# TheShinning/gps-sdr-sim

Hardware: AMD Instinct MI355X
Metric: IQ MSamples/s (and × real-time) at 2.6 MS/s, 12 sats, -b 16; 1/2/4/8 GPU (higher is better)
Workload: dtype int64 phases + f16 x f16 -> f32 MFMA accumulate (exact integer sums)

## Files before the change

### gps-sdr-sim_amd/csrc/common/gss_lin.h

```cpp
#ifndef GSS_LIN_H
#define GSS_LIN_H

#include <stdint.h>

#ifndef GSS_LIN_CH
#define GSS_LIN_CH     16
#endif
#define GSS_LIN_CHUNK  (64 * GSS_LIN_CH)
#define GSS_LIN_SEG    4096

#if defined(__HIPCC__)
#define GSS_LIN_FN static __host__ __device__ inline
#else
#define GSS_LIN_FN static inline
#endif

#define GSS_LIN_CSH    26

GSS_LIN_FN uint32_t gss_lin_dx(uint64_t xs) { return (uint32_t)((xs * 64u + (1ull << 31)) >> 32); }
GSS_LIN_FN uint32_t gss_lin_dz(uint64_t zs)
{
    return (uint32_t)((zs * 64u + (1ull << (GSS_LIN_CSH - 1))) >> GSS_LIN_CSH);
}
GSS_LIN_FN uint64_t gss_lin_xa(uint64_t xs)
{
    const int64_t e = (int64_t)(((uint64_t)gss_lin_dx(xs) << 32) - xs * 64u);
    return (1ull << 31) - (uint64_t)((e * (GSS_LIN_CH - 1)) / 2);
}
GSS_LIN_FN uint64_t gss_lin_za(uint64_t zs)
{
    const int64_t ec = (int64_t)(((uint64_t)gss_lin_dz(zs) << GSS_LIN_CSH) - zs * 64u);
    return (1ull << (GSS_LIN_CSH - 1)) - (uint64_t)((ec * (GSS_LIN_CH - 1)) / 2);
}

GSS_LIN_FN uint32_t gss_lin_e0(uint64_t chips)
{
    const uint32_t e = (uint32_t)(chips % 1023u);
    return e ? e : 1023u;
}

#define GSS_LIN_KDEV_CARR(zs)                                                                      \
    ((((uint64_t)GSS_LIN_CH / 2 + 3) << 31) +                                                     \
     ((2 + (((uint64_t)gss_lin_dz(zs) * (GSS_LIN_CH - 1)) >> 32)) << 32))
#define GSS_LIN_KDEV_CODE (((uint64_t)GSS_LIN_CH / 2 + 3) << (GSS_LIN_CSH - 1))
#define GSS_LIN_WIN_OK(zs) ((zs) * 63u + (3ull << 50) <= (31ull << 50))

#define GSS_LIN_TWE     2560
#define GSS_LIN_CBW_PRE 2
GSS_LIN_FN uint32_t gss_lin_wstep16(int n_per_blk)
{
    return (uint32_t)((104755200ull + (uint64_t)n_per_blk / 2) / (uint64_t)n_per_blk);
}
GSS_LIN_FN int gss_lin_win16_ok(uint64_t zs, int n_per_blk)
{
    const int64_t U = (int64_t)1 << 50, z = (int64_t)zs;
    const int64_t kd = (int64_t)GSS_LIN_KDEV_CODE + ((int64_t)1 << 27);
    const uint32_t w = gss_lin_wstep16(n_per_blk);
    if (zs == 0 || zs >= (uint64_t)U)
        return 0;
    for (int s = 0; s < GSS_LIN_CH; s++) {
        const int64_t f = (int64_t)(((uint64_t)s * w) >> 4) - GSS_LIN_CBW_PRE;
        if (64 * s * z - kd < f * U)
            return 0;
        if (U + (64 * s + 63) * z + kd > (f + 32) * U)
            return 0;
    }
    return 1025 * U + (int64_t)(GSS_LIN_SEG - GSS_LIN_CHUNK) * z + kd < (int64_t)GSS_LIN_TWE * U;
}

GSS_LIN_FN uint64_t gss_lin_lane(uint64_t xs, uint64_t zs, uint32_t l)
{
    const uint32_t lx = (uint32_t)(((uint64_t)l * xs + (1ull << 31)) >> 32);
    const uint32_t lz = (uint32_t)(((uint64_t)l * zs) >> GSS_LIN_CSH);
    return ((uint64_t)lx << 32) | lz;
}

typedef struct {
    int cell, chip;
} gss_lin_kc;

GSS_LIN_FN gss_lin_kc gss_lin_kernel_at(uint64_t x0, uint64_t xs, uint64_t z0, uint64_t zs,
                                         int64_t p)
{
    const int64_t c = p & ~(int64_t)(GSS_LIN_CHUNK - 1);
    const int64_t l = p & 63, s = (p - c) >> 6;
    const uint64_t lane = gss_lin_lane(xs, zs, (uint32_t)l);
    const int64_t n0 = p & ~(int64_t)(GSS_LIN_SEG - 1);
    const unsigned __int128 zn = (unsigned __int128)z0 + (unsigned __int128)(uint64_t)n0 * zs;
    const int64_t chips = (int64_t)(zn >> 50), e0 = gss_lin_e0((uint64_t)chips);
    const __int128 z = (__int128)z0 + (__int128)c * (__int128)zs -
                      (__int128)(chips - e0) * ((__int128)1 << 50);
    const unsigned __int128 zk = (unsigned __int128)((z + (int64_t)gss_lin_za(zs)) >> GSS_LIN_CSH);
    const uint64_t za = (uint64_t)(uint32_t)zk + (uint32_t)lane;
    const uint64_t zw = (uint64_t)(uint32_t)za + (uint64_t)s * gss_lin_dz(zs);
    const unsigned __int128 kz = zk + (uint32_t)lane + (unsigned __int128)(uint64_t)s *
                                 gss_lin_dz(zs);
    const uint32_t xb = (uint32_t)((x0 + (uint64_t)c * xs + gss_lin_xa(xs)) >> 32);
    const uint32_t xk = xb + (uint32_t)(lane >> 32) + (uint32_t)(za >> 32) +
                        (uint32_t)s * gss_lin_dx(xs) + (uint32_t)(zw >> 32);
    gss_lin_kc r;
    r.cell = (int)(xk >> 23);
    r.chip = (int)((uint64_t)(kz >> 24) % 1023u);
    return r;
}

#endif
```

### gps-sdr-sim_amd/csrc/hip/gss_synth.hip

```cpp
#include <hip/hip_runtime.h>
#include <stdint.h>
#include <stdlib.h>
#include <string.h>
#include "gpssim_amd.h"
#include "../common/gss_phase.h"
#include "../common/gss_lin.h"

#define SYNTH_THREADS  256
#define SYNTH_WAVES    (SYNTH_THREADS / 64)
#define ANCHOR_THREADS 64
#define CHUNK_BYTES    128
#define CHUNK_PIECES   (CHUNK_BYTES / 16)
#define LUT_N          1024

struct lut_arg { int16_t sin512[512]; int16_t cos512[512]; };

__global__ __launch_bounds__(ANCHOR_THREADS) void gss_anchor_kernel(
    const gss_chan_blk_t *__restrict__ blk, const int32_t *__restrict__ nch,
    const double *__restrict__ carr_ck, int nblk, int nchp, int n_per_blk, int nseg, int nsegp,
    int seg_r, double *__restrict__ seg_carr, double *__restrict__ seg_code,
    uint32_t *__restrict__ seg_cnt, double *__restrict__ carr_end,
    const int32_t *__restrict__ blist)
{
    const int nsub = carr_ck ? GSS_NCK : 1;
// ... 336 lines not shown
                if (src_full) {
                    uint8_t *sdst = dst + (ptrdiff_t)(src - lane) * ((ptrdiff_t)seg_r * BPS4 / 4) +
                                    (size_t)ch * CHUNK_BYTES + piece * 16;
                    const uint32_t *sp = stg + src * (CHUNK_BYTES / 4) + piece * 4;
                    store16(sdst, make_uint4(sp[0], sp[1], sp[2], sp[3]));
                }
            }
            wave_sync_lds();
        }
        if (!full && nsamp > 0) {
            int nbytes = nsamp * BPS4 / 4;
            uint8_t *bp = dst + (size_t)ch * CHUNK_BYTES;
            const uint8_t *sp = (const uint8_t *)mine;
            for (int i = 0; i < nbytes; i++)
                bp[i] = sp[i];
        }
    }
    if (bad && status)
        atomicOr(status, bad);
}

#define LIN_THREADS 256
#define LIN_WAVES   (LIN_THREADS / 64)
#define LIN_STEPS   (GSS_LIN_SEG / 64)
#define LIN_CH      GSS_LIN_CH
#define CBW_PRE     2
#define CBW_CHIPS   3072
#define CAB_W       ((CBW_CHIPS + 96) / 32)
static_assert(LIN_STEPS % LIN_CH == 0 && (LIN_CH & (LIN_CH - 1)) == 0, "whole chunks");
#define LIN_SW_SGPRS 68
typedef _Float16 lin_half4 __attribute__((ext_vector_type(4)));
typedef _Float16 lin_half8 __attribute__((ext_vector_type(8)));
typedef float lin_f4 __attribute__((ext_vector_type(4)));
#define LIN_GS    2
#define LIN_MAGF  (12582912.0f + 64.0f * LIN_GS)
#define LIN_MAGB  0x4B400000u

struct alignas(16) lin_ct {
    uint64_t B;
    uint64_t D;
    int32_t g;
    int32_t gd;
    int32_t pos1;
    uint32_t flags;
    uint32_t q0, dq, tab;
    uint32_t wa;
    uint32_t na, nb;
    uint32_t wn;
    uint32_t g2;
    uint32_t A[5][2];
};
static_assert(offsetof(lin_ct, A) % 8 == 0, "lin_ct.A: 8-byte reads");

struct lin_chan {
    uint64_t xs, zs;
    uint64_t d;
    uint32_t dq;
    uint32_t tab;
};
struct lin_seg {
    uint64_t x;
    uint64_t z;
    int32_t g01;
    int32_t pos1;
    uint32_t npatch;
    uint32_t pad;
};

__global__ void gss_linseg_kernel(const gss_lin_t *__restrict__ lin,
                                  const gss_chan_blk_t *__restrict__ blk,
                                  const int32_t *__restrict__ nch, const int32_t *__restrict__ fast,
                                  int nblk, int nseg, lin_seg *__restrict__ seg_out,
                                  lin_chan *__restrict__ chan_out)
{
    const int i = blockIdx.x * blockDim.x + threadIdx.x;
    if (i >= nblk * GSS_MAXCH * nseg)
        return;
    const int sg = i % nseg, bk = i / nseg, b = bk / GSS_MAXCH, k = bk % GSS_MAXCH;
    if (!fast[b] || k >= nch[b])
        return;
    const gss_lin_t *L = lin + bk;
    const uint64_t xa = gss_lin_xa(L->xs);
    if (sg == 0) {
        lin_chan c;
        c.xs = L->xs;
        c.zs = L->zs;
        c.d = ((uint64_t)gss_lin_dx(L->xs) << 32) | gss_lin_dz(L->zs);
        c.dq = (uint32_t)((L->zs * 64u) >> 46);
        c.tab = (uint32_t)blk[bk].ca_tbl;
        chan_out[bk] = c;
    }
    const uint64_t n0 = (uint64_t)sg * (64 * LIN_STEPS);
    const uint64_t lo = L->z0 + n0 * L->zs;
    const uint64_t hi = __umul64hi(n0, L->zs) + (lo < L->z0 ? 1u : 0u);
    const uint32_t E0 = gss_lin_e0((hi << 14) | (lo >> 50));
    lin_seg r;
    r.z = (((uint64_t)E0 << 50) | (lo & ((1ull << 50) - 1))) + gss_lin_za(L->zs);
    r.x = L->x0 + n0 * L->xs + xa;
    int q = 0;
    while (q + 1 < GSS_NGC && L->gpos[q + 1] <= (int)n0)
        q++;
    const int g0 = L->gval[q];
    const bool more = q + 1 < GSS_NGC && L->gpos[q + 1] < (int)n0 + 64 * LIN_STEPS;
    const int g1 = more ? L->gval[q + 1] : g0;
    r.g01 = (int32_t)(((uint32_t)g0 & 0xFFFFu) | ((uint32_t)g1 << 16));
    r.pos1 = more ? L->gpos[q + 1] : INT32_MAX;
    int np = 0;
    for (int j = 0; j < GSS_NPATCH; j++)
        np += L->ppos[j] >= (int)n0 && L->ppos[j] < (int)n0 + 64 * LIN_STEPS;
    r.npatch = (uint32_t)np;
    r.pad = 0;
    seg_out[i] = r;
}

__global__ void gss_cab_kernel(const uint32_t *__restrict__ ca_bits, int n_ca,
                               uint32_t *__restrict__ cab)
{
    const int i = blockIdx.x * blockDim.x + threadIdx.x;
    if (i >= n_ca * CAB_W)
        return;
    const int row = i / CAB_W, j0 = (i - row * CAB_W) * 32 - 32;
    const uint32_t *cb = ca_bits + (size_t)row * GSS_CA_WORDS;
    uint32_t w = 0;
    for (int q = 0; q < 32; q++) {
        const int e = j0 + q, chip = ((e % GSS_CA_LEN) + GSS_CA_LEN) % GSS_CA_LEN;
        w |= (((cb[chip >> 5] >> (chip & 31)) & 1u) ^ 1u) << q;
    }
    cab[i] = w;
}

__global__ void gss_tw16_kernel(const uint32_t *__restrict__ cab, int n_ca, uint32_t w,
                                uint32_t *__restrict__ tw)
{
    const int i = blockIdx.x * blockDim.x + threadIdx.x;
    if (i >= n_ca * GSS_LIN_TWE * LIN_CH)
        return;
    const int row = i / (GSS_LIN_TWE * LIN_CH), r = i - row * (GSS_LIN_TWE * LIN_CH);
    const int E = r / LIN_CH, st = r % LIN_CH;
    const uint32_t j = min((uint32_t)(E + (int)(((uint32_t)st * w) >> 4) - GSS_LIN_CBW_PRE + 32),
                           (uint32_t)(32 * CAB_W - 64));
    const uint32_t *c = cab + (size_t)row * CAB_W;
    const uint32_t lin = __builtin_amdgcn_alignbit(c[(j >> 5) + 1], c[j >> 5], j & 31);
    tw[i] = __builtin_amdgcn_alignbit(lin, lin, (32u - j) & 31u);
}

struct lin_wsrc {
    const uint32_t *W;
};

__device__ __forceinline__ void lin_wissue(const lin_wsrc &w, uint32_t (&ws)[LIN_CH])
{
#pragma unroll
    for (int s = 0; s < LIN_CH; s++)
        ws[s] = w.W[s];
}

__device__ __forceinline__ void lin_wfence(const uint32_t (&ws)[LIN_CH])
{
    static_assert(LIN_CH == 16, "the fence below names 16 windows");
    asm volatile("" :: "s"(ws[0]), "s"(ws[1]), "s"(ws[2]), "s"(ws[3]), "s"(ws[4]), "s"(ws[5]),
                 "s"(ws[6]), "s"(ws[7]), "s"(ws[8]), "s"(ws[9]), "s"(ws[10]), "s"(ws[11]),
                 "s"(ws[12]), "s"(ws[13]), "s"(ws[14]), "s"(ws[15]));
}

__device__ __forceinline__ lin_wsrc lin_wsrc_of(const lin_ct &t, const uint32_t *__restrict__ tw)
{
// ... 120 lines not shown
}

template <bool FIRST>
__device__ __forceinline__ void lin_sw_pair(lin_f4 (&cq)[LIN_CH / 2], lin_f4 c0, const lin_ct *T, int k0,
                                            int nc, int lane, const uint64_t *s_lane, uint32_t M,
                                            const int32_t *__restrict__ s_lut,
                                            const uint32_t *__restrict__ tw, uint32_t cls,
                                            bool more)
{
    const lin_ct &ta = T[k0], &tb = T[k0 + 1];
    uint64_t Pa = s_lane[k0 * 64 + lane] + ta.B, Pb = s_lane[(k0 + 1) * 64 + lane] + tb.B;
    const uint64_t Da = ta.D, Db = tb.D;
    const uint2 ga = *(const uint2 *)ta.A[cls], gb = *(const uint2 *)tb.A[cls];
    const lin_half8 A = __builtin_bit_cast(lin_half8, make_uint4(ga.x, ga.y, gb.x, gb.y));
    uint32_t na = ta.na, nb = ta.nb;
    asm volatile("" : "+v"(na), "+v"(nb));
    uint32_t wsa[LIN_CH], wsb[LIN_CH];
    lin_sw_take_a(wsa);
    lin_sw_take(wsb);
    if (k0 + 2 < nc || more)
        lin_sw_load2(tw, na, nb);
    uint32_t ea0 = 0, eb0 = 0;
#pragma unroll
    for (int s = 0; s < LIN_CH; s++) {
        uint32_t ta_, tb_;
        asm("v_lshrrev_b32_sdwa %0, %1, %2 dst_sel:DWORD dst_unused:UNUSED_PAD src0_sel:BYTE_3 "
            "src1_sel:DWORD" : "=v"(ta_) : "v"((uint32_t)Pa), "s"(wsa[s]));
        asm("v_lshrrev_b32_sdwa %0, %1, %2 dst_sel:DWORD dst_unused:UNUSED_PAD src0_sel:BYTE_3 "
            "src1_sel:DWORD" : "=v"(tb_) : "v"((uint32_t)Pb), "s"(wsb[s]));
        const uint32_t aa = __builtin_amdgcn_alignbit(ta_, (uint32_t)(Pa >> 32), 21) & M;
        const uint32_t ab = __builtin_amdgcn_alignbit(tb_, (uint32_t)(Pb >> 32), 21) & M;
        const uint32_t ea = *(const uint32_t *)((const char *)s_lut + aa);
        const uint32_t eb = *(const uint32_t *)((const char *)s_lut + ab);
        if (s & 1) {
            const uint4 bb = make_uint4(ea0, ea, eb0, eb);
            cq[s / 2] = __builtin_amdgcn_mfma_f32_16x16x32_f16(A, __builtin_bit_cast(lin_half8, bb),
                                                              FIRST ? c0 : cq[s / 2], 0, 0, 0);
        } else {
            ea0 = ea;
            eb0 = eb;
        }
        Pa += Da;
        Pb += Db;
    }
}

__device__ __forceinline__ lin_half4 lin_gain_operand(uint32_t gh, int lane)
{
    const uint32_t x = gh << ((lane & 1) * 16);
    const uint2 v = (lane & 2) ? make_uint2(0u, x) : make_uint2(x, 0u);
    return __builtin_bit_cast(lin_half4, v);
}

__device__ __forceinline__ uint32_t lin_f16_bits(int g)
{
    return (uint32_t)__builtin_bit_cast(uint16_t, (_Float16)(float)g);
}

__device__ __forceinline__ void lin_put(uint32_t *p, uint32_t v)
{
    __builtin_nontemporal_store(v, p);
}

extern "C" __device__ int gss_writelane(int, int, int) __asm("llvm.amdgcn.writelane.i32");

__device__ __forceinline__ uint32_t lin_ib(const lin_f4 (&cq)[LIN_CH / 2], int s)
{
    return __float_as_uint(cq[s / 2][2 * (s & 1)]);
}
__device__ __forceinline__ uint32_t lin_qb(const lin_f4 (&cq)[LIN_CH / 2], int s)
{
    return __float_as_uint(cq[s / 2][2 * (s & 1) + 1]);
}
__device__ __forceinline__ uint32_t lin_w16(const lin_f4 (&cq)[LIN_CH / 2], int s)
{
    const uint32_t pq = __builtin_amdgcn_perm(lin_qb(cq, s), lin_ib(cq, s), 0x06050201u);
    uint32_t r;
    asm("v_pk_add_u16 %0, %1, %2" : "=v"(r) : "v"(pq), "s"(0xC000C000u));
    return r;
}
__device__ __forceinline__ uint32_t lin_w8(const lin_f4 (&cq)[LIN_CH / 2], int s)
{
    constexpr uint32_t sh = 12u;
    uint32_t d = lin_ib(cq, s) >> sh;
    asm("v_lshrrev_b32_sdwa %0, %1, %2 dst_sel:BYTE_1 dst_unused:UNUSED_PRESERVE src0_sel:DWORD "
        "src1_sel:DWORD" : "+v"(d) : "v"(sh), "v"(lin_qb(cq, s)));
    return d;
}
__device__ __forceinline__ bool lin_ipos(const lin_f4 (&cq)[LIN_CH / 2], int s)
{
    return lin_ib(cq, s) >= LIN_MAGB + 128u * LIN_GS;
}
__device__ __forceinline__ bool lin_qpos(const lin_f4 (&cq)[LIN_CH / 2], int s)
{
    return lin_qb(cq, s) >= LIN_MAGB + 128u * LIN_GS;
}

template <int FMT, bool TAIL>
__device__ __forceinline__ void lin_store(const lin_f4 (&acc)[LIN_CH / 2], uint8_t *__restrict__ ob,
                                          int nb0, int lane, int n_per_blk)
{
    static_assert(FMT != 1 || LIN_CH == 16, "-b 1 packing assumes 16-step chunks");
    uint32_t pk[LIN_CH];
    pk[0] = 0;
#pragma unroll
    for (int s = 0; s < LIN_CH; s++) {
        const int nb = nb0 + s * 64, p = nb + lane;
// ... 40 lines not shown
                if (first + 4 * b < n_per_blk)
                    dst[b] = (uint8_t)(y >> (8 * b));
        }
    }
    if (FMT == 16) {
        __builtin_amdgcn_sched_barrier(0);
        if (!TAIL) {
            uint32_t *base = (uint32_t *)ob + nb0;
            const uint32_t off = (uint32_t)lane * 4u;
#pragma unroll
            for (int s = 0; s < LIN_CH; s++)
                asm volatile("global_store_dword %0, %1, %2 offset:%3 nt"
                             : : "v"(off), "v"(pk[s]), "s"(base + (s >> 4) * 1024),
                               "i"((s & 15) * 256) : "memory");
        } else {
#pragma unroll
            for (int s = 0; s < LIN_CH; s++) {
                const int p = nb0 + s * 64 + lane;
                if (!TAIL || p < n_per_blk)
                    lin_put(((uint32_t *)ob) + p, pk[s]);
            }
        }
    }
}

__device__ __forceinline__ void lin_patch_fix(lin_f4 (&cq)[LIN_CH / 2],
                                              const gss_lin_t *__restrict__ Lk, int nb0, int lane)
{
    for (int j = 0; j < GSS_NPATCH; j++) {
        const int pp = Lk->ppos[j];
        if (pp >= nb0 + 64 * LIN_CH)
            break;
        if (pp < nb0)
            continue;
        const int q = pp - nb0;
        const int64_t d = lane == (q & 63) ? Lk->pdelta[j] : 0;
        const int di = (int)((uint32_t)d << 10) >> 10;
        const float fi = (float)(di * LIN_GS), fq = (float)((int)((d - di) >> 22) * LIN_GS);
        const int sq = __builtin_amdgcn_readfirstlane(q >> 6);
#pragma unroll
        for (int s = 0; s < LIN_CH; s++) {
            const float m = s == sq ? 1.0f : 0.0f;
            cq[s / 2][2 * (s & 1)] = __builtin_fmaf(m, fi, cq[s / 2][2 * (s & 1)]);
            cq[s / 2][2 * (s & 1) + 1] = __builtin_fmaf(m, fq, cq[s / 2][2 * (s & 1) + 1]);
        }
    }
}


#define LIN_MINB 4
template <int FMT>
__global__ __launch_bounds__(LIN_THREADS, LIN_MINB) __attribute__((amdgpu_num_sgpr(LIN_SW_SGPRS)))
void gss_lin_kernel(
    const gss_lin_t *__restrict__ lin, const lin_seg *__restrict__ segs,
    const lin_chan *__restrict__ chans, const int32_t *__restrict__ nch,
    const int32_t *__restrict__ fast, const uint32_t *__restrict__ cab,
    const uint32_t *__restrict__ tw, lut_arg lut, int n_per_blk, int nseg, int wg_per_blk,
    uint8_t *__restrict__ out, size_t block_bytes)
{
    __shared__ int32_t s_lut[1024];
    __shared__ uint64_t s_lane[GSS_MAXCH * 64];
    __shared__ lin_ct s_ct[LIN_WAVES][GSS_MAXCH];
    const int b = blockIdx.x / wg_per_blk;
    const int w = blockIdx.x - b * wg_per_blk;
    if (!fast[b])
        return;
    const int tid = threadIdx.x, lane = tid & 63;
    const int wave = __builtin_amdgcn_readfirstlane(tid >> 6);
    for (int i = tid; i < 512; i += LIN_THREADS) {
        const uint32_t v = lin_f16_bits(lut.cos512[i]) | (lin_f16_bits(lut.sin512[i]) << 16);
        s_lut[i] = (int32_t)v;
        s_lut[512 + i] = (int32_t)(v ^ 0x80008000u);
    }
    const lin_chan *CH = chans + (size_t)b * GSS_MAXCH;
    const int nc = nch[b];
    for (int i = tid; i < nc * 64; i += LIN_THREADS)
        s_lane[i] = gss_lin_lane(CH[i >> 6].xs, CH[i >> 6].zs, (uint32_t)(i & 63));
    (void)cab;
    __syncthreads();
    uint32_t M = 0xFFCu;
    asm volatile("" : "+v"(M));
    const uint32_t cls = lin_pair_cls(lane);
    lin_f4 c0 = lin_f4{LIN_MAGF, LIN_MAGF, LIN_MAGF, LIN_MAGF};
    asm volatile("" : "+v"(c0));
    const int sg = w * LIN_WAVES + wave;
    const int n0 = sg * (64 * LIN_STEPS);
    if (n0 >= n_per_blk)
        return;
    const gss_lin_t *L = lin + (size_t)b * GSS_MAXCH;
    const lin_seg *S = segs + (size_t)b * GSS_MAXCH * nseg + sg;
    lin_ct *T = s_ct[wave];
    uint8_t *ob = out + (size_t)b * block_bytes;
    bool sw_ahead = false;
    uint64_t xb = 0, zb = 0, xs10 = 0, zs10 = 0;
    int32_t pos1 = INT32_MAX;
    uint32_t pflag = 0, gh0 = 0, gh1 = 0;
    uint32_t trow = 0, wa_next = 0;
    int g_after = -1;
    if (lane < nc) {
        const lin_chan ck = CH[lane];
        const lin_seg sk = S[(size_t)lane * nseg];
        xb = sk.x;
        zb = sk.z;
        xs10 = ck.xs << 10;
        zs10 = ck.zs << 10;
        static_assert(64 * LIN_CH == 1024, "one chunk = 2^10 samples");
        pos1 = sk.pos1;
        pflag = sk.npatch != 0 ? 2u : 0u;
        const int g0 = (int)(int16_t)(sk.g01 & 0xFFFF), g1 = sk.g01 >> 16;
        gh0 = lin_f16_bits(g0 * LIN_GS);
        gh1 = lin_f16_bits(g1 * LIN_GS);
        lin_ct &t = T[lane];
        t.D = ck.d;
        t.gd = g1 - g0;
        t.pos1 = sk.pos1;
        t.dq = ck.dq;
        t.tab = ck.tab;
        t.A[4][0] = 0;
        t.A[4][1] = 0;
        trow = ck.tab * GSS_LIN_TWE;
        wa_next = (trow + min((uint32_t)(zb >> 50), (uint32_t)(GSS_LIN_TWE - 1))) *
                  (uint32_t)(LIN_CH * sizeof(uint32_t));
    }

    const int nc_blk = nc;
    for (int c = 0; c < LIN_STEPS / LIN_CH; c++) {
        int nc = nc_blk;
        asm volatile("" : "+s"(nc));
        const int nb0 = n0 + c * (64 * LIN_CH);
        if (nb0 >= n_per_blk)
            break;
        const bool after = pos1 <= nb0;
        const bool chg = pos1 < nb0 + 64 * LIN_CH;
        const uint32_t my_flags = (chg && !after ? 1u : 0u) | pflag;
        const uint64_t zn = zb + zs10;
        const uint32_t my_wa = wa_next;
        const uint32_t my_wn = (trow + min((uint32_t)(zn >> 50), (uint32_t)(GSS_LIN_TWE - 1))) *
                               (uint32_t)(LIN_CH * sizeof(uint32_t));
        if (lane < nc) {
            lin_ct &t = T[lane];
            t.B = (xb & ~0xFFFFFFFFull) | (uint32_t)(zb >> GSS_LIN_CSH);
            t.flags = my_flags;
            t.wa = my_wa;
            t.wn = my_wn;
            if ((int)after != g_after) {
                g_after = (int)after;
                const uint32_t gh = after ? gh1 : gh0;
                t.A[0][0] = gh;         t.A[0][1] = 0;
                t.A[1][0] = gh << 16;   t.A[1][1] = 0;
                t.A[2][0] = 0;          t.A[2][1] = gh;
                t.A[3][0] = 0;          t.A[3][1] = gh << 16;
                t.g2 = gh | (gh << 16);
            }
        }
// ... 46 lines not shown
            lin_sw_take_a(ws);
            lin_sw_take(wb);
            (void)wb;
            if (more)
                lin_sw_load2(tw, wn0, wn1);
            lin_sw_steps(acc, T[k0], k0, lane, s_lane, M, s_lut, ws);
            k0 = nc;
        }
        sw_ahead = nc > 0 && more;
        for (int k = k0; k < nc; k++) {
            const lin_ct &t = T[k];
            const uint64_t B = t.B, D = t.D;
            const uint2 a2 = *(const uint2 *)t.A[lane & 3];
            lin_channel_chunk_m<false>(acc, c0, s_lane[k * 64 + lane] + B, D, lin_wsrc_of(t, tw), M,
                                       __builtin_bit_cast(lin_half4, a2), 0, 0, s_lut);
        }
        for (uint64_t fm = fmask; fm; fm &= fm - 1) {
            const int k = __builtin_amdgcn_readfirstlane((int)__builtin_ctzll(fm));
            const lin_ct &t = T[k];
            const uint64_t B = t.B, D = t.D;
            const uint32_t fl = __builtin_amdgcn_readfirstlane(t.flags);
            if (__builtin_expect(fl & 1u, 0)) {
                uint32_t l2 = (uint32_t)lane;
                asm volatile("" : "+v"(l2));
                lin_channel_chunk_m<true>(acc, c0, s_lane[k * 64 + l2] + B, D, lin_wsrc_of(t, tw), M,
                                          lin_gain_operand(lin_f16_bits(t.gd * LIN_GS), (int)l2), t.pos1,
                                          nb0 + (int)l2, s_lut);
            }
            if (__builtin_expect(fl & 2u, 0))
                lin_patch_fix(acc, L + k, nb0, lane);
        }
        wave_sync_lds();
        if (nb0 + 64 * LIN_CH <= n_per_blk)
            lin_store<FMT, false>(acc, ob, nb0, lane, n_per_blk);
        else
            lin_store<FMT, true>(acc, ob, nb0, lane, n_per_blk);
    }
}


struct gss_dev {
    int ordinal;
    int seg_r = 1024;
    struct anchor_set {
        double *carr = nullptr, *code = nullptr;
        uint32_t *cnt = nullptr;
        size_t cap = 0;
    } set[2];
    static constexpr int RING = 256;
    hipEvent_t ev_a[RING][2], ev_b[RING][2];
    hipEvent_t ev_l[RING][2];
    int n_a = 0, n_b = 0, n_l = 0;
    lut_arg lut;
    void *h_in = nullptr; size_t h_in_cap = 0;
    void *d_out = nullptr; size_t d_out_cap = 0;
    double *d_cend = nullptr; size_t d_cend_cap = 0;
    uint32_t *d_cbw = nullptr; size_t d_cbw_cap = 0;
    void *d_seg = nullptr; size_t d_seg_cap = 0;
    int32_t *d_status = nullptr;
    hipStream_t aux = nullptr;
    hipEvent_t ev_in = nullptr, ev_fb = nullptr;
};

extern "C" int gss_fail(int code, const char *fmt, ...);

#define HIP_TRY(x)                                                                           \
    do {                                                                                     \
        hipError_t e_ = (x);                                                                 \
        if (e_ != hipSuccess)                                                                \
            return gss_fail(GSS_E_HIP, "HIP error %s at %s:%d", hipGetErrorString(e_),      \
                            __FILE__, __LINE__);                                             \
    } while (0)

#define GSS_STR2(x) #x
#define GSS_STR(x) GSS_STR2(x)
extern "C" int gss_dev_ordinal(const gss_dev *d) { return d->ordinal; }

extern "C" const char *gss_build_info(void)
{
    return "lin_mfma=2 lin_ch=" GSS_STR(LIN_CH) " lin_swin=3 spec_k=" GSS_STR(GSS_SPEC_K)
           " arch=gfx950";
}


extern "C" void gss_run_pool_prewarm(int dev);

extern "C" int gss_dev_open(gss_dev **out, int ordinal)
{
    *out = nullptr;
    int count = 0;
    if (hipGetDeviceCount(&count) != hipSuccess || count <= 0)
        return gss_fail(GSS_E_NODEV, "no HIP device visible");
    if (ordinal < 0 || ordinal >= count)
        return gss_fail(GSS_E_ARG, "device ordinal %d out of range (%d devices)", ordinal, count);
    HIP_TRY(hipSetDevice(ordinal));
    gss_dev *d = new gss_dev();
    d->ordinal = ordinal;
    const char *r = getenv("GSS_SEG_R");
    if (r && atoi(r) >= 256 && atoi(r) % 256 == 0)
        d->seg_r = atoi(r);
    for (int i = 0; i < gss_dev::RING; i++)
        for (int j = 0; j < 2; j++) {
            HIP_TRY(hipEventCreate(&d->ev_a[i][j]));
            HIP_TRY(hipEventCreate(&d->ev_b[i][j]));
            HIP_TRY(hipEventCreate(&d->ev_l[i][j]));
        }
    int32_t s[512], c[512];
    gss_lut(s, c);
    for (int i = 0; i < 512; i++) {
        d->lut.sin512[i] = (int16_t)s[i];
        d->lut.cos512[i] = (int16_t)c[i];
    }
    HIP_TRY(hipMalloc(&d->d_status, sizeof(int32_t)));
    int prio_lo = 0, prio_hi = 0;
    HIP_TRY(hipDeviceGetStreamPriorityRange(&prio_lo, &prio_hi));
    HIP_TRY(hipStreamCreateWithPriority(&d->aux, hipStreamNonBlocking, prio_hi));
    HIP_TRY(hipEventCreateWithFlags(&d->ev_in, hipEventDisableTiming));
    HIP_TRY(hipEventCreateWithFlags(&d->ev_fb, hipEventDisableTiming));
    gss_run_pool_prewarm(ordinal);
    *out = d;
    return 0;
}

extern "C" void gss_run_pool_drain(int dev);

extern "C" int gss_dev_close(gss_dev *d)
{
    if (!d) return 0;
    (void)hipSetDevice(d->ordinal);
    gss_run_pool_drain(d->ordinal);
    for (auto &a : d->set) {
        (void)hipFree(a.carr);
        (void)hipFree(a.code);
        (void)hipFree(a.cnt);
    }
    if (d->aux) (void)hipStreamDestroy(d->aux);
    if (d->ev_in) (void)hipEventDestroy(d->ev_in);
    if (d->ev_fb) (void)hipEventDestroy(d->ev_fb);
    void *bufs[] = {d->h_in, d->d_out, d->d_cend, d->d_cbw, d->d_seg, d->d_status};
    for (void *p : bufs)
        (void)hipFree(p);
    for (int i = 0; i < gss_dev::RING; i++)
        for (int j = 0; j < 2; j++) {
            (void)hipEventDestroy(d->ev_a[i][j]);
            (void)hipEventDestroy(d->ev_b[i][j]);
            (void)hipEventDestroy(d->ev_l[i][j]);
        }
    delete d;
    return 0;
}

static int nseg_of(int n, int r) { return (n + r - 1) / r; }
static int nsegp_of(int n, int r) { return (nseg_of(n, r) + 1 + 31) & ~31; }

static int reserve_set(gss_dev *d, int set, int max_blocks, int n_per_blk, int R)
{
    gss_dev::anchor_set &a = d->set[set];
    size_t need = (size_t)max_blocks * GSS_MAXCH * (size_t)nsegp_of(n_per_blk, R);
    if (need <= a.cap)
        return 0;
    (void)hipFree(a.carr);
    (void)hipFree(a.code);
    (void)hipFree(a.cnt);
    a.carr = a.code = nullptr;
    a.cnt = nullptr;
    a.cap = 0;
    HIP_TRY(hipMalloc(&a.carr, need * sizeof(double)));
    HIP_TRY(hipMalloc(&a.code, need * sizeof(double)));
    HIP_TRY(hipMalloc(&a.cnt, need * sizeof(uint32_t)));
    a.cap = need;
    return 0;
}

extern "C" int gss_dev_reserve(gss_dev *d, int max_blocks, int n_per_blk)
{
    if (!d || max_blocks <= 0 || n_per_blk <= 0)
        return gss_fail(GSS_E_ARG, "invalid reserve arguments");
    HIP_TRY(hipSetDevice(d->ordinal));
    for (int set = 0; set < 2; set++) {
        int rc = reserve_set(d, set, max_blocks, n_per_blk, d->seg_r);
        if (rc) return rc;
    }
    return 0;
}

typedef void (*synth_fn)(const gss_chan_blk_t *, const int32_t *, const uint32_t *,
                         const uint32_t *, const double *, const double *, const uint32_t *,
                         lut_arg, int, int, int, int, int, uint8_t *, size_t, int32_t *,
                         const int32_t *);

template <int FMT> static synth_fn pick_nch(int nchp)
{
// ... 47 lines not shown
extern "C" int gss_anchor_device(gss_dev *d, int set, const gss_chan_blk_t *blk,
                                 const int32_t *nch, int nch_max, const double *carr_ck,
                                 int nblk, int n_per_blk, double *carr_end, void *stream)
{
    return anchor_launch(d, set, blk, nch, nch_max, carr_ck, nblk, n_per_blk, carr_end, nullptr,
                         d->seg_r, stream);
}

static int render_launch(gss_dev *d, int set, const gss_chan_blk_t *blk, const int32_t *nch,
                         int nch_max, const uint32_t *ca_bits, const uint32_t *nav, int nblk,
                         int n_per_blk, int fmt, void *out, int32_t *status,
                         const int32_t *blist, int R, void *stream)
{
    if (!d || !blk || !nch || !ca_bits || !out || nblk <= 0 || n_per_blk <= 0 || set < 0 ||
        set > 1)
        return gss_fail(GSS_E_ARG, "invalid render arguments");
    const size_t bb = gss_block_bytes(n_per_blk, fmt);
    if (bb == 0)
        return gss_fail(GSS_E_ARG, "invalid format %d for %d samples/block", fmt, n_per_blk);
    const int nseg = nseg_of(n_per_blk, R), nsegp = nsegp_of(n_per_blk, R);
    const gss_dev::anchor_set &a = d->set[set];
    if ((size_t)nblk * GSS_MAXCH * (size_t)nsegp > a.cap)
        return gss_fail(GSS_E_STATE, "anchor set %d holds no Stage A output of this size", set);
    const int nchp = nch_max < 1 ? 1 : nch_max;
    if (nchp > GSS_MAXCH)
        return gss_fail(GSS_E_ARG, "nch_max %d > %d", nch_max, GSS_MAXCH);
    synth_fn fn = pick_kernel(fmt, nchp);
    if (!fn)
        return gss_fail(GSS_E_ARG, "no kernel for fmt=%d nch=%d", fmt, nchp);
    HIP_TRY(hipSetDevice(d->ordinal));
    hipStream_t st = (hipStream_t)stream;
    hipEvent_t *ev = d->ev_b[d->n_b % gss_dev::RING];
    d->n_b++;
    const int wg_per_blk = (nseg + SYNTH_THREADS - 1) / SYNTH_THREADS;
    HIP_TRY(hipEventRecord(ev[0], st));
    hipLaunchKernelGGL(fn, dim3(nblk * wg_per_blk), dim3(SYNTH_THREADS), 0, st, blk, nch, ca_bits,
                       nav, a.carr, a.code, a.cnt, d->lut, n_per_blk, nseg, nsegp, R, wg_per_blk,
                       (uint8_t *)out, bb, status, blist);
    HIP_TRY(hipGetLastError());
    HIP_TRY(hipEventRecord(ev[1], st));
    return 0;
}

extern "C" int gss_render_device(gss_dev *d, int set, const gss_chan_blk_t *blk,
                                 const int32_t *nch, int nch_max, const uint32_t *ca_bits,
                                 int n_ca, const uint32_t *nav, int n_nav, int nblk,
                                 int n_per_blk, int fmt, void *out, int32_t *status, void *stream)
{
    (void)n_ca; (void)n_nav;
    return render_launch(d, set, blk, nch, nch_max, ca_bits, nav, nblk, n_per_blk, fmt, out,
                         status, nullptr, d->seg_r, stream);
}

typedef void (*lin_fn)(const gss_lin_t *, const lin_seg *, const lin_chan *, const int32_t *,
                       const int32_t *, const uint32_t *, const uint32_t *, lut_arg, int, int,
                       int, uint8_t *, size_t);

static lin_fn pick_lin(int fmt)
{
    switch (fmt) {
    case 16: return gss_lin_kernel<16>;
    case 8: return gss_lin_kernel<8>;
    case 1: return gss_lin_kernel<1>;
    default: return nullptr;
    }
}

extern "C" int gss_synth_lin_device(gss_dev *d, const gss_chan_blk_t *blk, const int32_t *nch,
                                    int nch_max, const gss_lin_t *lin, const int32_t *fast,
                                    const int32_t *fb_list, int n_fb, const double *carr_ck,
                                    const uint32_t *ca_bits, int n_ca, const uint32_t *nav,
                                    int n_nav, int nblk, int n_per_blk, int fmt, void *out,
                                    int32_t *status, void *stream)
{
    (void)n_nav;
    if (!d || !blk || !nch || !lin || !fast || !ca_bits || !out || nblk <= 0 || n_per_blk <= 0 ||
        n_ca <= 0 || n_fb < 0 || n_fb > nblk || (n_fb > 0 && !fb_list))
        return gss_fail(GSS_E_ARG, "invalid synth_lin arguments");
    const size_t bb = gss_block_bytes(n_per_blk, fmt);
    if (bb == 0)
        return gss_fail(GSS_E_ARG, "invalid format %d for %d samples/block", fmt, n_per_blk);
    const int nchp = nch_max < 1 ? 1 : nch_max;
    if (nchp > GSS_MAXCH)
        return gss_fail(GSS_E_ARG, "nch_max %d > %d", nch_max, GSS_MAXCH);
    lin_fn fn = pick_lin(fmt);
    if (!fn)
        return gss_fail(GSS_E_ARG, "no fast kernel for fmt=%d nch=%d", fmt, nchp);
    HIP_TRY(hipSetDevice(d->ordinal));
    hipStream_t st = (hipStream_t)stream;
    const size_t ncbw = (size_t)n_ca * CAB_W, ntw = (size_t)n_ca * GSS_LIN_TWE * LIN_CH;
    const size_t tw_off = (ncbw + 63) & ~(size_t)63;
    if ((tw_off + ntw) * sizeof(uint32_t) > d->d_cbw_cap) {
        (void)hipFree(d->d_cbw);
        d->d_cbw = nullptr;
        d->d_cbw_cap = 0;
        HIP_TRY(hipMalloc(&d->d_cbw, (tw_off + ntw) * sizeof(uint32_t)));
        d->d_cbw_cap = (tw_off + ntw) * sizeof(uint32_t);
    }
    hipLaunchKernelGGL(gss_cab_kernel, dim3((unsigned)((ncbw + 255) / 256)), dim3(256), 0, st,
                       ca_bits, n_ca, d->d_cbw);
    HIP_TRY(hipGetLastError());
    hipLaunchKernelGGL(gss_tw16_kernel, dim3((unsigned)((ntw + 255) / 256)), dim3(256), 0, st,
                       (const uint32_t *)d->d_cbw, n_ca, gss_lin_wstep16(n_per_blk),
                       d->d_cbw + tw_off);
    HIP_TRY(hipGetLastError());
    const int segs = (n_per_blk + 64 * LIN_STEPS - 1) / (64 * LIN_STEPS);
    const int wg_per_blk = (segs + LIN_WAVES - 1) / LIN_WAVES;
    const size_t nsegrows = (size_t)nblk * GSS_MAXCH * segs;
    const size_t seg_bytes = nsegrows * sizeof(lin_seg);
    const size_t need_rows = seg_bytes + (size_t)nblk * GSS_MAXCH * sizeof(lin_chan);
    if (need_rows > d->d_seg_cap) {
        (void)hipFree(d->d_seg);
        d->d_seg = nullptr;
        d->d_seg_cap = 0;
        HIP_TRY(hipMalloc(&d->d_seg, need_rows));
        d->d_seg_cap = need_rows;
    }
    lin_seg *d_segs = (lin_seg *)d->d_seg;
    lin_chan *d_chans = (lin_chan *)((char *)d->d_seg + seg_bytes);
    hipLaunchKernelGGL(gss_linseg_kernel, dim3((unsigned)((nsegrows + 255) / 256)), dim3(256), 0,
                       st, lin, blk, nch, fast, nblk, segs, d_segs, d_chans);
    HIP_TRY(hipGetLastError());
    if (n_fb > 0) {
        HIP_TRY(hipEventRecord(d->ev_in, st));
        HIP_TRY(hipStreamWaitEvent(d->aux, d->ev_in, 0));
        const int R = 256;
        int rc = anchor_launch(d, 0, blk, nch, nch_max, carr_ck, n_fb, n_per_blk, nullptr,
                               fb_list, R, d->aux);
        if (rc) return rc;
        rc = render_launch(d, 0, blk, nch, nch_max, ca_bits, nav, n_fb, n_per_blk, fmt, out,
                           status, fb_list, R, d->aux);
        if (rc) return rc;
        HIP_TRY(hipEventRecord(d->ev_fb, d->aux));
    }
    hipEvent_t *ev = d->ev_l[d->n_l % gss_dev::RING];
    d->n_l++;
    HIP_TRY(hipEventRecord(ev[0], st));
    hipLaunchKernelGGL(fn, dim3((unsigned)nblk * wg_per_blk), dim3(LIN_THREADS), 0, st, lin,
                       (const lin_seg *)d_segs, (const lin_chan *)d_chans, nch, fast, d->d_cbw,
                       d->d_cbw + tw_off, d->lut, n_per_blk, segs, wg_per_blk, (uint8_t *)out, bb);
    HIP_TRY(hipGetLastError());
    HIP_TRY(hipEventRecord(ev[1], st));
    if (n_fb > 0)
        HIP_TRY(hipStreamWaitEvent(st, d->ev_fb, 0));
    return 0;
}

extern "C" int gss_synth_device(gss_dev *d, const gss_chan_blk_t *blk, const int32_t *nch,
                                int nch_max, const double *carr_ck, const uint32_t *ca_bits,
                                int n_ca,
                                const uint32_t *nav, int n_nav, int nblk, int n_per_blk, int fmt,
                                void *out, double *carr_end, int32_t *status, void *stream)
{
    if (!d || !blk || !nch || !ca_bits || !out || nblk <= 0 || n_per_blk <= 0)
        return gss_fail(GSS_E_ARG, "invalid synth arguments");
    if (gss_block_bytes(n_per_blk, fmt) == 0)
        return gss_fail(GSS_E_ARG, "invalid format %d for %d samples/block", fmt, n_per_blk);
    int rc = gss_anchor_device(d, 0, blk, nch, nch_max, carr_ck, nblk, n_per_blk, carr_end,
                               stream);
    if (rc) return rc;
    return gss_render_device(d, 0, blk, nch, nch_max, ca_bits, n_ca, nav, n_nav, nblk, n_per_blk,
                             fmt, out, status, stream);
}

static int ring_avg(hipEvent_t (*ev)[2], int n, double *avg)
{
    const int cnt = n < gss_dev::RING ? n : gss_dev::RING;
    double acc = 0.0;
    if (cnt > 0) {
        HIP_TRY(hipEventSynchronize(ev[(n - 1) % gss_dev::RING][1]));
        for (int i = 0; i < cnt; i++) {
            hipEvent_t *e = ev[(n - 1 - i) % gss_dev::RING];
            float t = 0.f;
            HIP_TRY(hipEventElapsedTime(&t, e[0], e[1]));
            acc += t;
        }
        acc /= cnt;
    }
    *avg = acc;
    return 0;
}

extern "C" int gss_dev_timing(gss_dev *d, int reset, int *n, float *ckpt_ms, float *synth_ms)
{
    if (!d) return gss_fail(GSS_E_ARG, "null device");
    if (reset) {
        d->n_a = d->n_b = d->n_l = 0;
        return 0;
    }
    double a = 0.0, b = 0.0;
    int rc = ring_avg(d->ev_a, d->n_a, &a);
    if (rc) return rc;
    rc = ring_avg(d->ev_b, d->n_b, &b);
// ... 174 lines not shown
```

Measured before the change: 537,300.

## Fuse per-segment row setup into lin kernel and preload packed f16 LUT

Removes the separate gss_linseg_kernel launch and its global seg/chan buffers. Each workgroup now computes its own segment rows and channel constants into LDS, with the work split across waves. The f16 sin/cos LUT is packed once on the host at init and copied into LDS with a single 16-byte load per thread, replacing per-launch conversion. This saves a kernel launch and a global round trip per call, at the cost of some extra prologue work in every workgroup.

```diff
diff --git a/gps-sdr-sim_amd/csrc/common/gss_lin.h b/gps-sdr-sim_amd/csrc/common/gss_lin.h
--- a/gps-sdr-sim_amd/csrc/common/gss_lin.h
+++ b/gps-sdr-sim_amd/csrc/common/gss_lin.h
@@ -76,6 +76,89 @@
 }
 
 typedef struct {
+    uint64_t x;
+    uint64_t z;
+    int32_t g01;
+    int32_t pos1;
+    uint32_t npatch;
+    uint32_t pad;
+} gss_lin_row;
+typedef struct {
+    uint64_t xs, zs;
+    uint64_t d;
+    uint32_t dq;
+    uint32_t tab;
+} gss_lin_chan;
+
+GSS_LIN_FN uint64_t gss_lin_mulhi(uint64_t a, uint64_t b)
+{
+#if defined(__HIP_DEVICE_COMPILE__)
+    return __umul64hi(a, b);
+#else
+    return (uint64_t)(((unsigned __int128)a * b) >> 64);
+#endif
+}
+
+GSS_LIN_FN uint64_t gss_lin_row_x(uint64_t x0, uint64_t xs, uint64_t n0)
+{
+    return x0 + n0 * xs + gss_lin_xa(xs);
+}
+GSS_LIN_FN uint64_t gss_lin_row_z(uint64_t z0, uint64_t zs, uint64_t n0)
+{
+    const uint64_t lo = z0 + n0 * zs;
+    const uint64_t hi = gss_lin_mulhi(n0, zs) + (lo < z0 ? 1u : 0u);
+    const uint32_t e0 = gss_lin_e0((hi << 14) | (lo >> 50));
+    return (((uint64_t)e0 << 50) | (lo & ((1ull << 50) - 1))) + gss_lin_za(zs);
+}
+GSS_LIN_FN void gss_lin_row_gain(gss_lin_row *r, const int32_t *gpos, const int32_t *gval, int ngc,
+                                 int32_t n0)
+{
+    int32_t g0 = gval[0], gn = 0, pn = INT32_MAX;
+    for (int i = 1; i < ngc; i++) {
+        const int32_t p = gpos[i], v = gval[i];
+        g0 = p <= n0 ? v : g0;
+    }
+    for (int i = ngc - 1; i >= 1; i--) {
+        const int32_t p = gpos[i], v = gval[i];
+        gn = p > n0 ? v : gn;
+        pn = p > n0 ? p : pn;
+    }
+    const int more = pn < n0 + GSS_LIN_SEG;
+    const int32_t g1 = more ? gn : g0;
+    r->g01 = (int32_t)(((uint32_t)g0 & 0xFFFFu) | ((uint32_t)g1 << 16));
+    r->pos1 = more ? pn : INT32_MAX;
+}
+GSS_LIN_FN uint32_t gss_lin_row_npatch(const int32_t *ppos, int np, int32_t n0)
+{
+    uint32_t n = 0;
+    for (int j = 0; j < np; j++)
+        n += ppos[j] >= n0 && ppos[j] < n0 + GSS_LIN_SEG;
+    return n;
+}
+GSS_LIN_FN gss_lin_row gss_lin_row_at(uint64_t x0, uint64_t xs, uint64_t z0, uint64_t zs,
+                                      const int32_t *gpos, const int32_t *gval, int ngc,
+                                      const int32_t *ppos, int np, int32_t n0)
+{
+    gss_lin_row r;
+    r.x = gss_lin_row_x(x0, xs, (uint64_t)n0);
+    r.z = gss_lin_row_z(z0, zs, (uint64_t)n0);
+    gss_lin_row_gain(&r, gpos, gval, ngc, n0);
+    r.npatch = gss_lin_row_npatch(ppos, np, n0);
+    r.pad = 0;
+    return r;
+}
+GSS_LIN_FN gss_lin_chan gss_lin_chan_of(uint64_t xs, uint64_t zs, uint32_t ca_tbl)
+{
+    gss_lin_chan c;
+    c.xs = xs;
+    c.zs = zs;
+    c.d = ((uint64_t)gss_lin_dx(xs) << 32) | gss_lin_dz(zs);
+    c.dq = (uint32_t)((zs * 64u) >> 46);
+    c.tab = ca_tbl;
+    return c;
+}
+
+typedef struct {
     int cell, chip;
 } gss_lin_kc;
 
diff --git a/gps-sdr-sim_amd/csrc/hip/gss_synth.hip b/gps-sdr-sim_amd/csrc/hip/gss_synth.hip
--- a/gps-sdr-sim_amd/csrc/hip/gss_synth.hip
+++ b/gps-sdr-sim_amd/csrc/hip/gss_synth.hip
@@ -412,66 +412,9 @@
 };
 static_assert(offsetof(lin_ct, A) % 8 == 0, "lin_ct.A: 8-byte reads");
 
-struct lin_chan {
-    uint64_t xs, zs;
-    uint64_t d;
-    uint32_t dq;
-    uint32_t tab;
-};
-struct lin_seg {
-    uint64_t x;
-    uint64_t z;
-    int32_t g01;
-    int32_t pos1;
-    uint32_t npatch;
-    uint32_t pad;
-};
-
-__global__ void gss_linseg_kernel(const gss_lin_t *__restrict__ lin,
-                                  const gss_chan_blk_t *__restrict__ blk,
-                                  const int32_t *__restrict__ nch, const int32_t *__restrict__ fast,
-                                  int nblk, int nseg, lin_seg *__restrict__ seg_out,
-                                  lin_chan *__restrict__ chan_out)
-{
-    const int i = blockIdx.x * blockDim.x + threadIdx.x;
-    if (i >= nblk * GSS_MAXCH * nseg)
-        return;
-    const int sg = i % nseg, bk = i / nseg, b = bk / GSS_MAXCH, k = bk % GSS_MAXCH;
-    if (!fast[b] || k >= nch[b])
-        return;
-    const gss_lin_t *L = lin + bk;
-    const uint64_t xa = gss_lin_xa(L->xs);
-    if (sg == 0) {
-        lin_chan c;
-        c.xs = L->xs;
-        c.zs = L->zs;
-        c.d = ((uint64_t)gss_lin_dx(L->xs) << 32) | gss_lin_dz(L->zs);
-        c.dq = (uint32_t)((L->zs * 64u) >> 46);
-        c.tab = (uint32_t)blk[bk].ca_tbl;
-        chan_out[bk] = c;
-    }
-    const uint64_t n0 = (uint64_t)sg * (64 * LIN_STEPS);
-    const uint64_t lo = L->z0 + n0 * L->zs;
-    const uint64_t hi = __umul64hi(n0, L->zs) + (lo < L->z0 ? 1u : 0u);
-    const uint32_t E0 = gss_lin_e0((hi << 14) | (lo >> 50));
-    lin_seg r;
-    r.z = (((uint64_t)E0 << 50) | (lo & ((1ull << 50) - 1))) + gss_lin_za(L->zs);
-    r.x = L->x0 + n0 * L->xs + xa;
-    int q = 0;
-    while (q + 1 < GSS_NGC && L->gpos[q + 1] <= (int)n0)
-        q++;
-    const int g0 = L->gval[q];
-    const bool more = q + 1 < GSS_NGC && L->gpos[q + 1] < (int)n0 + 64 * LIN_STEPS;
-    const int g1 = more ? L->gval[q + 1] : g0;
-    r.g01 = (int32_t)(((uint32_t)g0 & 0xFFFFu) | ((uint32_t)g1 << 16));
-    r.pos1 = more ? L->gpos[q + 1] : INT32_MAX;
-    int np = 0;
-    for (int j = 0; j < GSS_NPATCH; j++)
-        np += L->ppos[j] >= (int)n0 && L->ppos[j] < (int)n0 + 64 * LIN_STEPS;
-    r.npatch = (uint32_t)np;
-    r.pad = 0;
-    seg_out[i] = r;
-}
+typedef gss_lin_row lin_seg;
+typedef gss_lin_chan lin_chan;
+static_assert(sizeof(lin_seg) == 32 && sizeof(lin_chan) == 32, "two 16-byte LDS reads each");
 
 __global__ void gss_cab_kernel(const uint32_t *__restrict__ ca_bits, int n_ca,
                                uint32_t *__restrict__ cab)
@@ -698,7 +641,7 @@
     return __builtin_bit_cast(lin_half4, v);
 }
 
-__device__ __forceinline__ uint32_t lin_f16_bits(int g)
+__host__ __device__ __forceinline__ uint32_t lin_f16_bits(int g)
 {
     return (uint32_t)__builtin_bit_cast(uint16_t, (_Float16)(float)g);
 }
@@ -845,30 +788,58 @@
 template <int FMT>
 __global__ __launch_bounds__(LIN_THREADS, LIN_MINB) __attribute__((amdgpu_num_sgpr(LIN_SW_SGPRS)))
 void gss_lin_kernel(
-    const gss_lin_t *__restrict__ lin, const lin_seg *__restrict__ segs,
-    const lin_chan *__restrict__ chans, const int32_t *__restrict__ nch,
-    const int32_t *__restrict__ fast, const uint32_t *__restrict__ cab,
-    const uint32_t *__restrict__ tw, lut_arg lut, int n_per_blk, int nseg, int wg_per_blk,
+    const gss_lin_t *__restrict__ lin, const gss_chan_blk_t *__restrict__ blk,
+    const int32_t *__restrict__ nch, const int32_t *__restrict__ fast,
+    const uint32_t *__restrict__ cab, const uint32_t *__restrict__ tw,
+    const uint4 *__restrict__ lut16, int n_per_blk, int wg_per_blk,
     uint8_t *__restrict__ out, size_t block_bytes)
 {
-    __shared__ int32_t s_lut[1024];
+    __shared__ alignas(16) int32_t s_lut[1024];
     __shared__ uint64_t s_lane[GSS_MAXCH * 64];
     __shared__ lin_ct s_ct[LIN_WAVES][GSS_MAXCH];
+    __shared__ alignas(16) lin_seg s_seg[LIN_WAVES][GSS_MAXCH];
+    __shared__ alignas(16) lin_chan s_chan[GSS_MAXCH];
     const int b = blockIdx.x / wg_per_blk;
     const int w = blockIdx.x - b * wg_per_blk;
     if (!fast[b])
         return;
     const int tid = threadIdx.x, lane = tid & 63;
     const int wave = __builtin_amdgcn_readfirstlane(tid >> 6);
-    for (int i = tid; i < 512; i += LIN_THREADS) {
-        const uint32_t v = lin_f16_bits(lut.cos512[i]) | (lin_f16_bits(lut.sin512[i]) << 16);
-        s_lut[i] = (int32_t)v;
-        s_lut[512 + i] = (int32_t)(v ^ 0x80008000u);
-    }
-    const lin_chan *CH = chans + (size_t)b * GSS_MAXCH;
+    static_assert(sizeof(s_lut) == LIN_THREADS * sizeof(uint4), "one 16-byte copy per thread");
+    const uint4 lutv = lut16[tid];
+    const gss_lin_t *L = lin + (size_t)b * GSS_MAXCH;
     const int nc = nch[b];
-    for (int i = tid; i < nc * 64; i += LIN_THREADS)
-        s_lane[i] = gss_lin_lane(CH[i >> 6].xs, CH[i >> 6].zs, (uint32_t)(i & 63));
+#pragma unroll
+    for (int j = 0; j < GSS_MAXCH / LIN_WAVES; j++) {
+        const int k = wave + j * LIN_WAVES;
+        if (k < nc)
+            s_lane[k * 64 + lane] = gss_lin_lane(L[k].xs, L[k].zs, (uint32_t)lane);
+    }
+    {
+        const int rk = lane & (GSS_MAXCH - 1), rj = lane / GSS_MAXCH;
+        static_assert(LIN_WAVES * GSS_MAXCH == 64 && LIN_WAVES == 4, "one row per lane, 4 parts");
+        const int rn0 = (w * LIN_WAVES + rj) * (64 * LIN_STEPS);
+        if (rk < nc && rn0 < n_per_blk) {
+            const gss_lin_t *Lk = L + rk;
+            lin_seg &r = s_seg[rj][rk];
+            if (wave == 0) {
+                r.x = gss_lin_row_x(Lk->x0, Lk->xs, (uint64_t)rn0);
+                r.z = gss_lin_row_z(Lk->z0, Lk->zs, (uint64_t)rn0);
+            } else if (wave == 1) {
+                gss_lin_row g;
+                gss_lin_row_gain(&g, Lk->gpos, Lk->gval, GSS_NGC, rn0);
+                r.g01 = g.g01;
+                r.pos1 = g.pos1;
+            } else if (wave == 2) {
+                r.npatch = gss_lin_row_npatch(Lk->ppos, GSS_NPATCH, rn0);
+                r.pad = 0;
+            } else if (rj == 0) {
+                s_chan[rk] = gss_lin_chan_of(Lk->xs, Lk->zs,
+                                             (uint32_t)blk[(size_t)b * GSS_MAXCH + rk].ca_tbl);
+            }
+        }
+    }
+    ((uint4 *)s_lut)[tid] = lutv;
     (void)cab;
     __syncthreads();
     uint32_t M = 0xFFCu;
@@ -880,8 +851,6 @@
     const int n0 = sg * (64 * LIN_STEPS);
     if (n0 >= n_per_blk)
         return;
-    const gss_lin_t *L = lin + (size_t)b * GSS_MAXCH;
-    const lin_seg *S = segs + (size_t)b * GSS_MAXCH * nseg + sg;
     lin_ct *T = s_ct[wave];
     uint8_t *ob = out + (size_t)b * block_bytes;
     bool sw_ahead = false;
@@ -891,8 +860,8 @@
     uint32_t trow = 0, wa_next = 0;
     int g_after = -1;
     if (lane < nc) {
-        const lin_chan ck = CH[lane];
-        const lin_seg sk = S[(size_t)lane * nseg];
+        const lin_chan ck = s_chan[lane];
+        const lin_seg sk = s_seg[wave][lane];
         xb = sk.x;
         zb = sk.z;
         xs10 = ck.xs << 10;
@@ -1045,11 +1014,11 @@
     hipEvent_t ev_l[RING][2];
     int n_a = 0, n_b = 0, n_l = 0;
     lut_arg lut;
+    uint4 *d_lut16 = nullptr;
     void *h_in = nullptr; size_t h_in_cap = 0;
     void *d_out = nullptr; size_t d_out_cap = 0;
     double *d_cend = nullptr; size_t d_cend_cap = 0;
     uint32_t *d_cbw = nullptr; size_t d_cbw_cap = 0;
-    void *d_seg = nullptr; size_t d_seg_cap = 0;
     int32_t *d_status = nullptr;
     hipStream_t aux = nullptr;
     hipEvent_t ev_in = nullptr, ev_fb = nullptr;
@@ -1104,6 +1073,16 @@
         d->lut.sin512[i] = (int16_t)s[i];
         d->lut.cos512[i] = (int16_t)c[i];
     }
+    {
+        uint32_t packed[1024];
+        for (int i = 0; i < 512; i++) {
+            const uint32_t v = lin_f16_bits(c[i]) | (lin_f16_bits(s[i]) << 16);
+            packed[i] = v;
+            packed[512 + i] = v ^ 0x80008000u;
+        }
+        HIP_TRY(hipMalloc(&d->d_lut16, sizeof(packed)));
+        HIP_TRY(hipMemcpy(d->d_lut16, packed, sizeof(packed), hipMemcpyHostToDevice));
+    }
     HIP_TRY(hipMalloc(&d->d_status, sizeof(int32_t)));
     int prio_lo = 0, prio_hi = 0;
     HIP_TRY(hipDeviceGetStreamPriorityRange(&prio_lo, &prio_hi));
@@ -1130,7 +1109,7 @@
     if (d->aux) (void)hipStreamDestroy(d->aux);
     if (d->ev_in) (void)hipEventDestroy(d->ev_in);
     if (d->ev_fb) (void)hipEventDestroy(d->ev_fb);
-    void *bufs[] = {d->h_in, d->d_out, d->d_cend, d->d_cbw, d->d_seg, d->d_status};
+    void *bufs[] = {d->h_in, d->d_out, d->d_cend, d->d_cbw, d->d_lut16, d->d_status};
     for (void *p : bufs)
         (void)hipFree(p);
     for (int i = 0; i < gss_dev::RING; i++)
@@ -1284,8 +1263,8 @@
                          status, nullptr, d->seg_r, stream);
 }
 
-typedef void (*lin_fn)(const gss_lin_t *, const lin_seg *, const lin_chan *, const int32_t *,
-                       const int32_t *, const uint32_t *, const uint32_t *, lut_arg, int, int,
+typedef void (*lin_fn)(const gss_lin_t *, const gss_chan_blk_t *, const int32_t *,
+                       const int32_t *, const uint32_t *, const uint32_t *, const uint4 *, int,
                        int, uint8_t *, size_t);
 
 static lin_fn pick_lin(int fmt)
@@ -1338,21 +1317,6 @@
     HIP_TRY(hipGetLastError());
     const int segs = (n_per_blk + 64 * LIN_STEPS - 1) / (64 * LIN_STEPS);
     const int wg_per_blk = (segs + LIN_WAVES - 1) / LIN_WAVES;
-    const size_t nsegrows = (size_t)nblk * GSS_MAXCH * segs;
-    const size_t seg_bytes = nsegrows * sizeof(lin_seg);
-    const size_t need_rows = seg_bytes + (size_t)nblk * GSS_MAXCH * sizeof(lin_chan);
-    if (need_rows > d->d_seg_cap) {
-        (void)hipFree(d->d_seg);
-        d->d_seg = nullptr;
-        d->d_seg_cap = 0;
-        HIP_TRY(hipMalloc(&d->d_seg, need_rows));
-        d->d_seg_cap = need_rows;
-    }
-    lin_seg *d_segs = (lin_seg *)d->d_seg;
-    lin_chan *d_chans = (lin_chan *)((char *)d->d_seg + seg_bytes);
-    hipLaunchKernelGGL(gss_linseg_kernel, dim3((unsigned)((nsegrows + 255) / 256)), dim3(256), 0,
-                       st, lin, blk, nch, fast, nblk, segs, d_segs, d_chans);
-    HIP_TRY(hipGetLastError());
     if (n_fb > 0) {
         HIP_TRY(hipEventRecord(d->ev_in, st));
         HIP_TRY(hipStreamWaitEvent(d->aux, d->ev_in, 0));
@@ -1369,8 +1333,8 @@
     d->n_l++;
     HIP_TRY(hipEventRecord(ev[0], st));
     hipLaunchKernelGGL(fn, dim3((unsigned)nblk * wg_per_blk), dim3(LIN_THREADS), 0, st, lin,
-                       (const lin_seg *)d_segs, (const lin_chan *)d_chans, nch, fast, d->d_cbw,
-                       d->d_cbw + tw_off, d->lut, n_per_blk, segs, wg_per_blk, (uint8_t *)out, bb);
+                       blk, nch, fast, d->d_cbw, d->d_cbw + tw_off, (const uint4 *)d->d_lut16,
+                       n_per_blk, wg_per_blk, (uint8_t *)out, bb);
     HIP_TRY(hipGetLastError());
     HIP_TRY(hipEventRecord(ev[1], st));
     if (n_fb > 0)
```

New measurement: 543,700, median of 6. 1.2% higher.
